# beilsme/rs-image-segmentation

Measured on AMD Instinct MI355X. Metric: Mpixel/s feature-extract+classify, higher is better.
Workload: dtype f32

## Files before the change

### profiles/code_object_diff.py

```python
#!/usr/bin/env python3
import json
import os
import re
import subprocess
import sys
import tempfile
from concurrent.futures import ThreadPoolExecutor

HIPCC = os.environ.get("HIPCC", "/opt/rocm/bin/hipcc")


def makefile_flags(csrc):
    text = open(os.path.join(csrc, "Makefile")).read()
    arch = re.search(r"^ARCH \?= *(\S+)", text, re.M).group(1)
    return re.search(r"^CXXFLAGS \?= *(.*)$", text, re.M).group(1).replace("$(ARCH)", arch).split()


def asm(csrc, f, tmp, tag):
    out = os.path.join(tmp, f"{tag}_{f}.s")
    subprocess.check_call([HIPCC, *makefile_flags(csrc), "--cuda-device-only", "-S", f, "-o", out], cwd=csrc, stderr=subprocess.DEVNULL)
    return open(out).read()


def demangle(names):
    p = subprocess.run(["c++filt"], input="\n".join(names), capture_output=True, text=True)
    return dict(zip(names, p.stdout.split("\n")))


def kernels(text):
    res = {}
    for m in re.finditer(r"^(\w+):\s*; @\1\n(.*?)^\s*\.end_amdhsa_kernel", text, re.S | re.M):
        ins = [ln.split(";")[0].strip() for ln in m.group(2).split("\n")]
        res[m.group(1)] = {"ins": [i for i in ins if i and not i.startswith(".")]}
    for m in re.finditer(r"- \.agpr_count:.*?\.name:\s+(\w+).*?\.wavefront_size", text, re.S):
        blk, name = m.group(0), m.group(1)
        if name in res:
            for key, field in (("vgprs", "vgpr_count"), ("agprs", "agpr_count"), ("sgprs", "sgpr_count"), ("lds", "group_segment_fixed_size"),
                               ("scratch", "private_segment_fixed_size"), ("wg", "max_flat_workgroup_size")):
                res[name][key] = int(re.search(r"\." + field + r":\s+(\d+)", blk).group(1))
    return res


def waves_per_simd(k):
    regs = -(-k["vgprs"] // 8) * 8 + -(-k["agprs"] // 8) * 8
    w = min(8, 512 // max(regs, 8))
    if k["lds"]:
        w = min(w, (160 * 1024 // k["lds"]) * -(-k["wg"] // 64) // 4)
    return w


def main():
    parent, new, outp, files = sys.argv[1], sys.argv[2], sys.argv[3], sys.argv[4:]
    table = []
    with tempfile.TemporaryDirectory() as tmp, ThreadPoolExecutor(8) as ex:
        jobs = {(t, f): ex.submit(asm, c, f, tmp, t) for f in files for t, c in (("parent", parent), ("new", new))
                if os.path.exists(os.path.join(c, f))}
        for f in files:
            if ("parent", f) not in jobs:
                kn = kernels(jobs[("new", f)].result())
                names = demangle(sorted(kn))
                for name in sorted(kn):
                    b = kn[name]
                    row = {"file": f, "kernel": names[name].split("(")[0].replace("void ", ""), "new_file": True}
                    for k in ("vgprs", "sgprs", "lds", "scratch"):
                        row[k] = [None, b[k]]
                    row["waves_per_simd"] = [None, waves_per_simd(b)]
                    row["instructions"] = [None, len(b["ins"])]
                    row["identical"] = None
                    row["within_the_rules"] = b["scratch"] == 0
                    table.append(row)
                    print("new  " + ("" if row["within_the_rules"] else "RULE ") + json.dumps(row))
                continue
            kp, kn = kernels(jobs[("parent", f)].result()), kernels(jobs[("new", f)].result())
            assert set(kp) == set(kn), (f, set(kp) ^ set(kn))
            names = demangle(sorted(kp))
            for name in sorted(kp):
                a, b = kp[name], kn[name]
                row = {"file": f, "kernel": names[name].split("(")[0].replace("void ", "")}
                for k in ("vgprs", "sgprs", "lds", "scratch"):
                    row[k] = [a[k], b[k]]
                row["waves_per_simd"] = [waves_per_simd(a), waves_per_simd(b)]
                row["instructions"] = [len(a["ins"]), len(b["ins"])]
                row["identical"] = a["ins"] == b["ins"]
                row["within_the_rules"] = b["scratch"] == 0 and a["lds"] == b["lds"] and row["waves_per_simd"][1] >= row["waves_per_simd"][0]
                table.append(row)
                print(("same " if row["identical"] else "DIFF ") + ("" if row["within_the_rules"] else "RULE ") + json.dumps(row))
    json.dump(table, open(outp, "w"), indent=1)


main()
```

### rs-image-segmentation_amd/csrc/k9_kmeans.hip

```cpp
#include <algorithm>
#include <chrono>
#include <cmath>
#include <type_traits>

#include "common.h"
#include "k9_kmeans.h"

template <typename T> constexpr bool lloyd_pipelined(int KMAX, int FR, bool UPDATE) { return KMAX <= 32 && (UPDATE || FR >= 16); }
template <typename T> constexpr bool kpp_pipelined(int NL, int FR) { return true; }
template <typename T> __device__ __forceinline__ int km_full_tiles(int64_t chunk0, int64_t n)
{
    const int64_t left = n - chunk0;
    if (left <= 0) return 0;
    const int64_t full = left / km_tile<T>();
    return full < KM_TILES_PER_CHUNK ? (int)full : KM_TILES_PER_CHUNK;
}

template <typename T>
__global__ __launch_bounds__(KM_THREADS) void km_minmax(planes_t pl, int64_t n, T *__restrict__ pmin, T *__restrict__ pmax)
{
    constexpr int PXL = vt<T>::PXL;
    const int f = blockIdx.y;
    T mn = (T)INFINITY, mx = (T)-INFINITY;
    for (int64_t base = ((int64_t)blockIdx.x * KM_THREADS + threadIdx.x) * PXL; base < n; base += (int64_t)gridDim.x * KM_THREADS * PXL) {
        T v[PXL];
// ... 48 lines not shown
            base += UNR * stride;
            if (!fits(base)) { consume(va); break; }
            request(vb, base);
            consume(va);
            base += UNR * stride;
            if (!fits(base)) { consume(vb); break; }
            request(va, base);
            consume(vb);
        }
    }
    for (; base < n; base += stride) {
        T v[PXL];
        load_px<T>(pl.p[f], base, n, v);
#pragma unroll
        for (int i = 0; i < PXL; i++)
            if (base + i < n) acc += to_fixed40((double)scaled<T>(v[i], sc, mnv));
    }
    __shared__ long long sacc[4];
    wg_put(sacc, wave_sum(acc));
    __syncthreads();
    if (threadIdx.x == 0) partial[(size_t)f * gridDim.x + blockIdx.x] = wg_sum(sacc);
}

template <typename T>
__global__ void km_gather_row(planes_t pl, int F, int64_t idx, const scaler_t<T> *__restrict__ sp, T *__restrict__ out)
{
    const int f = threadIdx.x;
    if (f < F) {
        T x = reinterpret_cast<const T *>(pl.p[f])[idx];
        out[f] = scaled<T>(x, sp->scale[f], sp->minv[f]) - sp->mean[f];
    }
}

#define KPP_MAXL 8
#define KPP_STRIDE (KPP_MAXL + 1)

template <typename T> __device__ __forceinline__ T kpp_close(double dot, double cc, double yy)
{
    double d = -2.0 * dot;
    d = d + cc;
    d = d + yy;
    const T dt = (T)d;
    return dt > (T)0 ? dt : (T)0;
}

template <typename T, int NL, int FR, int MODE>
__global__ __launch_bounds__(KM_THREADS) void km_kpp(planes_t pl, int F, int64_t n, const scaler_t<T> *__restrict__ sp,
                                                     const double *__restrict__ candT, const double *__restrict__ cc, int L,
                                                     T *__restrict__ closest, unsigned long long *__restrict__ partial, int64_t nchunks,
                                                     int store)
{
    constexpr int PXL = vt<T>::PXL;
    constexpr bool VAR = MODE == 0;
    constexpr bool PIPE = kpp_pipelined<T>(NL, FR);
    unsigned long long acc[NL];
#pragma unroll
    for (int l = 0; l < NL; l++) acc[l] = 0;
    long long vacc[VAR ? FR : 1];
#pragma unroll
    for (int f = 0; f < (VAR ? FR : 1); f++) vacc[f] = 0;
    const int64_t chunk0 = (int64_t)blockIdx.x * km_chunk<T>();
    auto request = [&](T (&x)[FR][PXL], T (&cl)[PXL], uint32_t off) {
#pragma unroll
        for (int f = 0; f < FR; f++) load_pxq<T>(pl, F, f, chunk0, off, x[f]);
        if constexpr (MODE == 2) load_pxf<T, true>(closest, chunk0 + off, n, cl);
    };
    auto tile_body = [&](auto full_t, auto roll_c, T (&x)[FR][PXL], T (&cl)[PXL], uint32_t off, uint32_t noff) {
        const int64_t base = chunk0 + off;
        constexpr bool FULL = decltype(full_t)::value;
        constexpr int ROLL = decltype(roll_c)::value;
        static_assert(ROLL == 0 || FULL, "only full tiles are requested ahead");
        if constexpr (ROLL == 0) {
#pragma unroll
            for (int f = 0; f < FR; f++) {
                if (f < F) load_pxf<T, FULL>(pl.p[f], base, n, x[f]);
                else {
#pragma unroll
                    for (int p = 0; p < PXL; p++) x[f][p] = (T)0;
                }
            }
#pragma unroll
            for (int p = 0; p < PXL; p++) cl[p] = (T)0;
            if constexpr (MODE == 2) load_pxf<T, FULL>(closest, base, n, cl);
        }
        double dot[NL][PXL], dotp[PXL], yy[PXL];
#pragma unroll
        for (int p = 0; p < PXL; p++) {
            yy[p] = 0.0;
            dotp[p] = 0.0;
#pragma unroll
            for (int l = 0; l < NL; l++) dot[l][p] = 0.0;
        }
#pragma unroll
        for (int f = 0; f < FR; f++) {
            if (f < F) {
                const T sc = sp->scale[f], mnv = sp->minv[f], me = sp->mean[f];
                double cd[NL];
#pragma unroll
                for (int l = 0; l < NL; l++) cd[l] = candT[f * KPP_STRIDE + l];
                const double cdp = candT[f * KPP_STRIDE + KPP_MAXL];
#pragma unroll
                for (int p = 0; p < PXL; p++) {
                    const T yt = scaled<T>(x[f][p], sc, mnv) - me;
                    if constexpr (VAR) {
                        const T dd = yt * yt;
                        if (FULL || base + p < n) vacc[f] += to_fixed40((double)dd);
                    }
                    const double y = (double)yt;
                    yy[p] = fma(y, y, yy[p]);
                    if constexpr (MODE != 0) dotp[p] = fma(cdp, y, dotp[p]);
#pragma unroll
                    for (int l = 0; l < NL; l++) dot[l][p] = fma(cd[l], y, dot[l][p]);
                }
            }
            if constexpr (ROLL == 1) load_pxq<T>(pl, F, f, chunk0, noff, x[f]);
        }
        if constexpr (MODE != 0) {
            const double ccp = cc[KPP_MAXL];
            bool moved = MODE != 2;
#pragma unroll
            for (int p = 0; p < PXL; p++) {
                T dt = kpp_close<T>(dotp[p], ccp, yy[p]);
                if constexpr (MODE == 2) {
                    moved = moved || dt < cl[p];
                    dt = cl[p] < dt ? cl[p] : dt;
                }
                cl[p] = dt;
            }
            if (!store) {
            } else if (FULL || base + PXL <= n) {
                if (moved) {
                    typename vt<T>::vec o;
                    if constexpr (PXL == 4) o = make_float4(cl[0], cl[1], cl[2], cl[3]);
                    else o = make_double2(cl[0], cl[1]);
                    *reinterpret_cast<typename vt<T>::vec *>(closest + base) = o;
                }
            } else {
                for (int p = 0; p < PXL; p++)
                    if (base + p < n) closest[base + p] = cl[p];
            }
        }
#pragma unroll
        for (int l = 0; l < NL; l++) {
            if (l < L) {
                const double ccl = cc[l];
#pragma unroll
                for (int p = 0; p < PXL; p++) {
                    T dt = kpp_close<T>(dot[l][p], ccl, yy[p]);
                    if constexpr (MODE != 0) dt = cl[p] < dt ? cl[p] : dt;
                    if (FULL || base + p < n) acc[l] += (unsigned long long)to_fixed40((double)dt);
                }
            }
        }
        if constexpr (ROLL == 1 && MODE == 2) load_pxf<T, true>(closest, chunk0 + noff, n, cl);
    };
    T x[FR][PXL], cl[PXL];
    auto at = [&](int t) { return (uint32_t)(t * km_tile<T>() + (int)threadIdx.x * PXL); };
    if constexpr (!PIPE) {
        for (int t = 0; t < KM_TILES_PER_CHUNK; t++) {
            const int64_t tbase = chunk0 + (int64_t)t * km_tile<T>();
            if (tbase >= n) break;
            if (tbase + km_tile<T>() <= n) tile_body(std::true_type{}, ic<0>(), x, cl, at(t), 0);
            else tile_body(std::false_type{}, ic<0>(), x, cl, at(t), 0);
        }
    } else {
        const int nfull = km_full_tiles<T>(chunk0, n);
        if (nfull > 0) {
            request(x, cl, at(0));
#pragma clang loop unroll(disable)
            for (int t = 0; t + 1 < nfull; t++) tile_body(std::true_type{}, ic<1>(), x, cl, at(t), at(t + 1));
            tile_body(std::true_type{}, ic<2>(), x, cl, at(nfull - 1), 0);
        }
        if (nfull < KM_TILES_PER_CHUNK && chunk0 + (int64_t)nfull * km_tile<T>() < n) tile_body(std::false_type{}, ic<0>(), x, cl, at(nfull), 0);
    }
    __shared__ unsigned long long sacc[4][NL];
#pragma unroll
    for (int l = 0; l < NL; l++) {
// ... 9 lines not shown
#pragma unroll
        for (int f = 0; f < FR; f++) {
            long long s = wave_sum(vacc[f]);
            if (lane_id() == 0) svar[threadIdx.x >> 6][f] = s;
        }
        __syncthreads();
        if ((int)threadIdx.x < F)
            partial[(size_t)(1 + threadIdx.x) * nchunks + blockIdx.x] =
                (unsigned long long)(svar[0][threadIdx.x] + svar[1][threadIdx.x] + svar[2][threadIdx.x] + svar[3][threadIdx.x]);
    }
}

struct kpp_sample_args {
    int64_t c0[KPP_MAXL], cn[KPP_MAXL], direct[KPP_MAXL];
    unsigned long long rem[KPP_MAXL];
    int mode[KPP_MAXL];
    int with_old;
    int64_t offset;
};
template <typename T>
__global__ __launch_bounds__(KM_THREADS) void km_kpp_chunkq(planes_t pl, int F, const scaler_t<T> *__restrict__ sp,
                                                            const double *__restrict__ candT, const double *__restrict__ cc,
                                                            const T *__restrict__ closest, const kpp_sample_args *__restrict__ ap,
                                                            unsigned long long *__restrict__ qv)
{
    const kpp_sample_args &a = *ap;
    const int l = blockIdx.y;
    if (a.mode[l] != 1) return;
    const int64_t c0 = a.c0[l], cn = a.cn[l];
    const int64_t i = (int64_t)blockIdx.x * KM_THREADS + threadIdx.x;
    if (i >= cn) return;
    const double ccp = cc[KPP_MAXL];
    double yy = 0.0, dotp = 0.0;
    for (int f = 0; f < F; f++) {
        const T xv = reinterpret_cast<const T *>(pl.p[f])[c0 + i];
        const T yt = scaled<T>(xv, sp->scale[f], sp->minv[f]) - sp->mean[f];
        const double y = (double)yt;
        yy = fma(y, y, yy);
        dotp = fma(candT[f * KPP_STRIDE + KPP_MAXL], y, dotp);
    }
    T dt = kpp_close<T>(dotp, ccp, yy);
    if (a.with_old) {
        const T c = closest[c0 + i];
        dt = c < dt ? c : dt;
    }
    qv[(size_t)l * km_chunk<T>() + i] = (unsigned long long)to_fixed40((double)dt);
}

template <typename T>
__global__ __launch_bounds__(KM_THREADS) void km_kpp_sample(planes_t pl, int F, const scaler_t<T> *__restrict__ sp,
                                                            const unsigned long long *__restrict__ qv, const kpp_sample_args *__restrict__ ap,
                                                            double *__restrict__ out)
{
    const kpp_sample_args &a = *ap;
// ... 782 lines not shown
    if (be == 0) e = -1074;
    else { m |= 1ull << 52; e = be - 1075; }
    const int sft = e + 40;
    if (sft >= 0) return (u128)m << sft;
    const int sh = -sft;
    if (sh >= 64) return (u128)1;
    const unsigned long long q = m >> sh, rem = m & ((1ull << sh) - 1ull);
    return (u128)q + (rem ? 1 : 0);
}

template <typename T>
__global__ __launch_bounds__(64) void kc_mean_pack(const km_state<T> *__restrict__ st, const T *__restrict__ row, int own0, long long *__restrict__ x)
{
    const int F = st->F, f = threadIdx.x;
    if (f >= F) return;
    if (st->n_local <= 0) { x[2 * f] = 0; x[2 * f + 1] = 0; }
    double rv = own0 ? (double)row[f] : 0.0;
    if (rv == 0.0) rv = 0.0;
    x[2 * F + f] = __double_as_longlong(rv);
}

template <typename T>
__global__ __launch_bounds__(KM_THREADS) void kc_mean_apply(km_state<T> *__restrict__ st, scaler_t<T> *__restrict__ sp, const long long *__restrict__ x,
                                                            double *__restrict__ candT)
{
    const int F = st->F;
    double *cc = candT + (size_t)KPP_STRIDE * RSSEG_MAX_FEATURES;
    for (int i = threadIdx.x; i < KPP_STRIDE * RSSEG_MAX_FEATURES + KPP_STRIDE; i += KM_THREADS) candT[i] = 0.0;
    __syncthreads();
    const T Nt = (T)st->N;
    if ((int)threadIdx.x < F) {
        const int f = threadIdx.x;
        const T sT = fixed_to_T<T>(limbs(x[2 * f], x[2 * f + 1]));
        const T m = sT / Nt;
        sp->mean[f] = m;
        st->mean[f] = m;
        const T raw = (T)__longlong_as_double(x[2 * F + f]);
        const T c0 = raw - m;
        st->C[0][f] = c0;
        candT[f * KPP_STRIDE] = (double)c0;
    }
    __syncthreads();
    if (threadIdx.x == 0) {
        double a = 0.0;
        for (int f = 0; f < F; f++) a = fma((double)st->C[0][f], (double)st->C[0][f], a);
        cc[0] = a;
    }
}

template <typename T>
__global__ __launch_bounds__(KM_THREADS) void kc_tol(km_state<T> *__restrict__ st, const long long *__restrict__ x)
{
    __shared__ T var[RSSEG_MAX_FEATURES];
    const int F = st->F;
    const T Nt = (T)st->N;
    if ((int)threadIdx.x < F) {
        const T sT = fixed_to_T<T>(limbs(x[2 * threadIdx.x], x[2 * threadIdx.x + 1]));
        var[threadIdx.x] = sT / Nt;
    }
    __syncthreads();
    if (threadIdx.x == 0) {
        const T m = np_pairwise_sum<T>(var, F);
        const T m2 = m / (T)F;
        st->tol = m2 * (T)st->tol_in;
        u128 total = 0;
        for (int r = 0; r < st->world; r++) {
            st->rank_tot[r] = kc_ulimbs(x[2 * F + 2 * r], x[2 * F + 2 * r + 1]);
            total += st->rank_tot[r];
        }
        st->current_pot = (T)((double)total * (1.0 / 1099511627776.0));
        st->best = 0;
    }
}

template <typename T> __device__ __forceinline__ void kc_pick_body(km_state<T> *st, int c, const long long *x);

template <typename T>
__global__ __launch_bounds__(KM_THREADS) void kc_targets(km_state<T> *st, int c, int pick_c, const unsigned long long *__restrict__ part,
                                                         double *__restrict__ candT, kpp_sample_args *__restrict__ sa_out, double *xbuf, long long *lim)
{
    if (pick_c > 0) kc_pick_body<T>(st, pick_c, lim);
    for (int i = threadIdx.x; i < KPP_MAXL * (1 + RSSEG_MAX_FEATURES); i += KM_THREADS) xbuf[i] = 0.0;
    for (int i = threadIdx.x; i < 2 * KPP_MAXL * RSSEG_MAX_RANKS; i += KM_THREADS)
        if (i < 2 * st->L * st->world) lim[i] = 0;
    const int F = st->F, L = st->L;
    double *cc = candT + (size_t)KPP_STRIDE * RSSEG_MAX_FEATURES;
    for (int i = threadIdx.x; i < KPP_STRIDE * RSSEG_MAX_FEATURES + KPP_STRIDE; i += KM_THREADS) candT[i] = 0.0;
    __syncthreads();
    if ((int)threadIdx.x < F) candT[threadIdx.x * KPP_STRIDE + KPP_MAXL] = (double)st->C[c - 1][threadIdx.x];
    if (threadIdx.x == 0) {
        double a = 0.0;
        for (int f = 0; f < F; f++) a = fma((double)st->C[c - 1][f], (double)st->C[c - 1][f], a);
        cc[KPP_MAXL] = a;
    }
    __shared__ kpp_sample_args sa;
    __shared__ u128 ssum[KM_THREADS];
    __shared__ u128 gsum[16];
    for (int i = threadIdx.x; i < (int)(sizeof(sa) / 4); i += KM_THREADS) reinterpret_cast<int *>(&sa)[i] = 0;
    const long long nchunks = st->nchunks, n = st->n_local;
    const unsigned long long *pre = part + (size_t)st->best * nchunks;
    const long long slice = (nchunks + KM_THREADS - 1) / KM_THREADS;
    {
        u128 mine = 0;
        const long long c_lo = (long long)threadIdx.x * slice, c_hi = c_lo + slice < nchunks ? c_lo + slice : nchunks;
        if (n > 0) {
            long long ch = c_lo;
            for (; ch + 8 <= c_hi; ch += 8) {
                unsigned long long v[8];
#pragma unroll
                for (int u = 0; u < 8; u++) v[u] = pre[ch + u];
#pragma unroll
                for (int u = 0; u < 8; u++) mine += v[u];
            }
            for (; ch < c_hi; ch++) mine += pre[ch];
        }
        ssum[threadIdx.x] = mine;
// ... 223 lines not shown
                if (update) {
                    RSCHK(set_max_dyn_lds(ctx, (const void *)km_lloyd_blk<T, KM, true>, lds));
                    hipLaunchKernelGGL((km_lloyd_blk<T, KM, true>), grid, block, lds, ctx->stream, pl, F, k, n, sp, cenT, csq, labels, partial,
                                       nchunks, ncopies, done);
                } else {
                    hipLaunchKernelGGL((km_lloyd_blk<T, KM, false>), grid, block, 0, ctx->stream, pl, F, k, n, sp, cenT, csq, labels, partial,
                                       nchunks, ncopies, done);
                }
            } else {
                if (update) {
                    RSCHK(set_max_dyn_lds(ctx, (const void *)km_lloyd<T, KM, FR, true>, lds));
                    hipLaunchKernelGGL((km_lloyd<T, KM, FR, true>), grid, block, lds, ctx->stream, pl, F, k, n, sp, cenT, csq, labels, partial,
                                       nchunks, ncopies, done, (int32_t *)nullptr);
                } else {
                    hipLaunchKernelGGL((km_lloyd<T, KM, FR, false>), grid, block, 0, ctx->stream, pl, F, k, n, sp, cenT, csq, labels, partial,
                                       nchunks, ncopies, done, out32);
                }
            }
            return RSSEG_OK;
        });
    });
}

template <typename T>
void launch_kpp(rsseg_ctx *ctx, int64_t nchunks, planes_t pl, int F, int64_t n, const scaler_t<T> *sp, const double *cand, const double *cc,
                int L, int mode, bool last, T *closest, unsigned long long *partial)
{
    auto go = [&](auto nl_c, auto mode_c) {
        constexpr int NL = decltype(nl_c)::value, MODE = decltype(mode_c)::value;
        with_width(km_width(F), [&](auto fr_c) {
            constexpr int FR = decltype(fr_c)::value;
            const dim3 grid((unsigned)nchunks), block(KM_THREADS);
            if constexpr (FR != KM_BLOCKED) {
                hipLaunchKernelGGL((km_kpp<T, NL, FR, MODE>), grid, block, 0, ctx->stream, pl, F, n, sp, cand, cc, L, closest, partial, nchunks,
                                   last ? 0 : 1);
            } else {
                hipLaunchKernelGGL((km_kpp_blk<T, NL, MODE>), grid, block, 0, ctx->stream, pl, F, n, sp, cand, cc, L, closest, partial, nchunks,
                                   last ? 0 : 1);
                if constexpr (MODE == 0)
                    hipLaunchKernelGGL((km_var<T>), dim3((unsigned)nchunks, F), block, 0, ctx->stream, pl, n, sp, partial, nchunks);
            }
        });
    };
    if (mode == 0) go(ic<1>(), ic<0>());
    else if (L <= 4) mode == 1 ? go(ic<4>(), ic<1>()) : go(ic<4>(), ic<2>());
    else mode == 1 ? go(ic<8>(), ic<1>()) : go(ic<8>(), ic<2>());
}

template <typename T>
void launch_farthest(rsseg_ctx *ctx, int KMAX, int64_t nchunks, planes_t pl, int F, int64_t n, int64_t offset, const scaler_t<T> *sp,
                     const T *cenT, const uint8_t *labels, const taken_t &tk, T *pdist, long long *pidx)
{
    with_kmax(KMAX, [&](auto kmax_c) {
        with_width(km_width(F), [&](auto fr_c) {
            hipLaunchKernelGGL((km_farthest<T, decltype(kmax_c)::value, decltype(fr_c)::value>), dim3((unsigned)nchunks), dim3(KM_THREADS), 0,
                               ctx->stream, pl, F, n, offset, sp, cenT, labels, tk, pdist, pidx);
        });
    });
}

constexpr size_t LIM_OFF = ((sizeof(double) * KPP_MAXL * (1 + RSSEG_MAX_FEATURES)) + 511) & ~(size_t)511;
constexpr size_t UP_SLOT = 64 * 1024;

template <typename T> struct km_fit {
    static constexpr int CHUNK = km_chunk<T>();
    rsseg_ctx *ctx = nullptr;
    hipStream_t st = nullptr;
    planes_t pl;
    int max_iter = 0;
    int F = 0, k = 0, KMAX = 0, L = 0, M = 0, nblk = 0;
    int64_t n = 0, nchunks = 0, N = 0, offset = 0;
    int64_t n_all[RSSEG_MAX_RANKS] = {0};
    int last_rank = 0;
    struct {
        scaler_t<T> *sp;
        T *cen, *csq;
        double *cand, *cc;
        T *row;
        unsigned long long *qv;
        long long *red;
        kpp_sample_args *sa;
        long long *redsave;
        km_state<T> *lst;
        T *mm;
        long long *mom, *part;
        T *closest;
        uint8_t *lab;
    } d;
    long long *x = nullptr;
    size_t pin_main = 0;
    unsigned up_i = 0, up_since_sync = 0;
    long long up_epoch = 0;
    int ncopies = KM_COPIES;
    size_t lds = 0;
    scaler_t<T> sp;
    T C[RSSEG_MAX_CLUSTERS][RSSEG_MAX_FEATURES];
    int64_t init_idx[RSSEG_MAX_CLUSTERS];
    T tol = (T)0;
    int it = 0, relocated = 0;
    bool strict = false;

    int setup(rsseg_ctx *c, int F_, int64_t n_, int k_, int max_iter_)
    {
        ctx = c;
        st = c->stream;
        F = F_, n = n_, k = k_, max_iter = max_iter_;
        KMAX = km_kmax(k);
        L = 2 + (int)std::log((double)k);
        if (L > KPP_MAXL) return rs_fail(ctx, RSSEG_ERR_UNSUPPORTED, "kmeans: too many local trials");
        M = KMAX * F + KMAX + 1;
        nchunks = std::max<int64_t>(1, ceil_div64(n, CHUNK));
        nblk = (int)std::min<int64_t>(2048, std::max<int64_t>(1, ceil_div64(n, (int64_t)KM_THREADS * vt<T>::PXL)));
        while (ncopies > 1 && sizeof(long long) * (size_t)ncopies * km_copy_stride(KMAX, F) > 48 * 1024) ncopies >>= 1;
        lds = sizeof(long long) * (size_t)ncopies * km_copy_stride(KMAX, F);
        if (lds > 150 * 1024) return rs_fail(ctx, RSSEG_ERR_UNSUPPORTED, "kmeans: F=%d, k=%d needs %zu B of LDS", F, k, lds);
        return RSSEG_OK;
    }

    int layout(const void *const *d_planes)
    {
        const size_t x_bytes = sizeof(long long) * std::max<size_t>({(size_t)2 * M, (size_t)3 * F, (size_t)2 * F + 2 * (size_t)ctx->world,
                                                                     LIM_OFF / sizeof(long long) + 2 * (size_t)L * ctx->world});
        if (ctx->comm_on && x_bytes > ctx->comm_bytes) return rs_fail(ctx, RSSEG_ERR_COMM, "kmeans: comm buffer too small (%zu > %zu)", x_bytes, ctx->comm_bytes);
        size_t off = 0;
        auto carve = [&](size_t bytes) { size_t o = off; off = (off + bytes + 255) & ~(size_t)255; return o; };
        const size_t o_sp = carve(sizeof(scaler_t<T>));
        const size_t o_cen = carve(sizeof(T) * ((size_t)KMAX * RSSEG_MAX_FEATURES + KMAX));
        const size_t o_cand = carve(sizeof(double) * ((size_t)KPP_STRIDE * RSSEG_MAX_FEATURES + KPP_STRIDE));
        const size_t o_row = carve(sizeof(T) * RSSEG_MAX_FEATURES);
        const size_t o_qv = carve(sizeof(unsigned long long) * KPP_MAXL * (size_t)CHUNK);
        const size_t o_red = carve(x_bytes);
        const size_t o_sa = carve(sizeof(kpp_sample_args));
        const size_t o_redsave = carve(sizeof(long long) * 2 * M);
        const size_t o_lst = carve(sizeof(km_state<T>));
        const size_t o_mm = carve(sizeof(T) * 2 * (size_t)nblk * F);
        const size_t o_mom = carve(sizeof(long long) * (size_t)nblk * F);
        const size_t o_part = carve(sizeof(long long) * std::max<size_t>((size_t)M, KPP_MAXL) * (size_t)nchunks);
        const size_t o_closest = carve((sizeof(T) * (size_t)std::max<int64_t>(n, 1) + 255) & ~(size_t)255);
        const size_t o_lab = carve((size_t)std::max<int64_t>(n, 1) + 64);
        RSCHK(ws_reserve(ctx, off));
        char *ws = ctx->d_ws;
        d.sp = (scaler_t<T> *)(ws + o_sp);
        d.cen = (T *)(ws + o_cen);
        d.csq = d.cen + (size_t)KMAX * RSSEG_MAX_FEATURES;
        d.cand = (double *)(ws + o_cand);
        d.cc = d.cand + (size_t)KPP_STRIDE * RSSEG_MAX_FEATURES;
        d.row = (T *)(ws + o_row);
        d.qv = (unsigned long long *)(ws + o_qv);
        d.red = (long long *)(ws + o_red);
        d.sa = (kpp_sample_args *)(ws + o_sa);
        d.redsave = (long long *)(ws + o_redsave);
        d.lst = (km_state<T> *)(ws + o_lst);
        d.mm = (T *)(ws + o_mm);
        d.mom = (long long *)(ws + o_mom);
        d.part = (long long *)(ws + o_part);
        d.closest = (T *)(ws + o_closest);
        d.lab = (uint8_t *)(ws + o_lab);
        x = ctx->comm_on ? (long long *)ctx->d_comm : d.red;
        const size_t pin_need = std::max<size_t>({sizeof(T) * 2 * (size_t)nblk * F, sizeof(long long) * (size_t)nblk * F + sizeof(double) * RSSEG_MAX_FEATURES + 64,
                                                  sizeof(long long) * (size_t)std::max(KPP_MAXL, F + 1) * (size_t)nchunks, sizeof(T) * (size_t)CHUNK,
                                                  sizeof(long long) * 2 * (size_t)M + sizeof(km_state<T>), (size_t)65536});
        pin_main = (pin_need + 255) & ~(size_t)255;
        RSCHK(pin_reserve(ctx, pin_main + 4 * UP_SLOT));
        up_epoch = ctx->host_syncs;
        memset(&pl, 0, sizeof(pl));
        for (int f = 0; f < F; f++) {
            if (n > 0 && (!d_planes[f] || ((uintptr_t)d_planes[f] & 15))) return rs_fail(ctx, RSSEG_ERR_INVALID, "kmeans: plane %d null or not 16-byte aligned", f);
            pl.p[f] = d_planes[f];
        }
        return RSSEG_OK;
    }

    hipError_t upload(void *dst, const void *src, size_t bytes)
    {
        if (ctx->host_syncs != up_epoch) { up_epoch = ctx->host_syncs; up_since_sync = 0; }
        if (up_since_sync == 4) {
            const hipError_t e = rs_sync(ctx);
            if (e != hipSuccess) return e;
            up_epoch = ctx->host_syncs;
// ... 58 lines not shown
    {
        {
            mt19937 rng(seed);
            km_state<T> hs;
            memset(&hs, 0, sizeof(hs));
            const double u0 = rng.random_sample();
            init_idx[0] = uniform_choice(N, std::is_same<T, float>::value ? RSSEG_F32 : RSSEG_F64, u0);
            if (init_idx[0] >= N) init_idx[0] = N - 1;
            for (int i = 0; i < (k - 1) * L; i++) hs.uniforms[i] = rng.random_sample();
            hs.init_idx[0] = init_idx[0];
            hs.max_iter = max_iter;
            for (int r = 0; r < ctx->world; r++) hs.n_all[r] = n_all[r];
            hs.N = N; hs.offset = offset; hs.n_local = n; hs.nchunks = nchunks;
            hs.rank = ctx->rank; hs.world = ctx->world; hs.k = k; hs.F = F; hs.L = L; hs.last_rank = last_rank;
            hs.tol_in = tol_in;
            static_assert(sizeof(hs) <= UP_SLOT, "upload slot too small");
            HIPCHK(ctx, upload(d.lst, &hs, sizeof(hs)));
        }
        const int64_t li0 = init_idx[0] - offset;
        const bool own0 = li0 >= 0 && li0 < n;
        if (n > 0) {
            {
                prof_scope ps(ctx, "moment");
                hipLaunchKernelGGL((km_moment<T>), dim3(nblk, F), dim3(KM_THREADS), 0, st, pl, n, d.sp, d.mom);
            }
            if (own0) hipLaunchKernelGGL((km_gather_row<T>), dim3(1), dim3(64), 0, st, pl, F, li0, d.sp, d.row);
            hipLaunchKernelGGL(km_reduce_cols, dim3(F), dim3(KM_THREADS), 0, st, (const long long *)d.mom, (int64_t)nblk, x, (const int *)nullptr, 1, 0);
        }
        hipLaunchKernelGGL((kc_mean_pack<T>), dim3(1), dim3(64), 0, st, (const km_state<T> *)d.lst, (const T *)d.row, own0 ? 1 : 0, x);
        HIPCHK(ctx, hipGetLastError());
        RSCHK(comm_allreduce_dev(ctx, 0, 3 * F, RSSEG_I64, RSSEG_SUM));
        hipLaunchKernelGGL((kc_mean_apply<T>), dim3(1), dim3(KM_THREADS), 0, st, d.lst, d.sp, (const long long *)x, d.cand);
        HIPCHK(ctx, hipGetLastError());
        return RSSEG_OK;
    }

    int kpp_rounds()
    {
        if (n > 0) {
            prof_scope ps(ctx, "kpp");
            launch_kpp<T>(ctx, nchunks, pl, F, n, d.sp, d.cand, d.cc, 1, 0, false, d.closest, (unsigned long long *)d.part);
        }
        HIPCHK(ctx, hipGetLastError());
        HIPCHK(ctx, hipMemsetAsync(x, 0, sizeof(long long) * (2 * (size_t)F + 2 * (size_t)ctx->world), st));
        if (n > 0) {
            hipLaunchKernelGGL(km_reduce_cols, dim3(F), dim3(KM_THREADS), 0, st, (const long long *)d.part + nchunks, nchunks, x, (const int *)nullptr, 1, 0);
            hipLaunchKernelGGL(km_reduce_cols, dim3(1), dim3(KM_THREADS), 0, st, (const long long *)d.part, nchunks, x + 2 * F, (const int *)nullptr, 1, ctx->rank);
        }
        HIPCHK(ctx, hipGetLastError());
        RSCHK(comm_allreduce_dev(ctx, 0, 2 * F + 2 * ctx->world, RSSEG_I64, RSSEG_SUM));
        hipLaunchKernelGGL((kc_tol<T>), dim3(1), dim3(KM_THREADS), 0, st, d.lst, (const long long *)x);
        HIPCHK(ctx, hipGetLastError());
        double *xbuf = (double *)x;
        long long *lim = (long long *)((char *)x + LIM_OFF);
        for (int c = 1; c < k; c++) {
            hipLaunchKernelGGL((kc_targets<T>), dim3(1), dim3(KM_THREADS), 0, st, d.lst, c, c > 1 ? c - 1 : 0, (const unsigned long long *)d.part, d.cand, d.sa,
                               xbuf, lim);
            if (n > 0) {
                hipLaunchKernelGGL((km_kpp_chunkq<T>), dim3((unsigned)(CHUNK / KM_THREADS), L), dim3(KM_THREADS), 0, st, pl, F, d.sp, d.cand, d.cc,
                                   (const T *)d.closest, (const kpp_sample_args *)d.sa, d.qv);
                hipLaunchKernelGGL((km_kpp_sample<T>), dim3(L), dim3(KM_THREADS), 0, st, pl, F, d.sp, (const unsigned long long *)d.qv, (const kpp_sample_args *)d.sa, xbuf);
            }
            HIPCHK(ctx, hipGetLastError());
            RSCHK(comm_allreduce_dev(ctx, 0, (int64_t)L * (1 + RSSEG_MAX_FEATURES), RSSEG_F64, RSSEG_SUM));
            hipLaunchKernelGGL((kc_cands<T>), dim3(1), dim3(KM_THREADS), 0, st, d.lst, (const double *)xbuf, d.cand);
            if (n > 0) {
                prof_scope ps(ctx, "kpp");
                launch_kpp<T>(ctx, nchunks, pl, F, n, d.sp, d.cand, d.cc, L, c > 1 ? 2 : 1, c == k - 1, d.closest, (unsigned long long *)d.part);
            }
            HIPCHK(ctx, hipGetLastError());
            if (n > 0) hipLaunchKernelGGL(km_reduce_cols, dim3(L), dim3(KM_THREADS), 0, st, (const long long *)d.part, nchunks, lim, (const int *)nullptr, ctx->world, ctx->rank);
            RSCHK(comm_allreduce_dev(ctx, (int64_t)LIM_OFF, 2 * (int64_t)L * ctx->world, RSSEG_I64, RSSEG_SUM));
        }
        if (k > 1) {
            hipLaunchKernelGGL((kc_pick<T>), dim3(1), dim3(KM_THREADS), 0, st, d.lst, k - 1, (const long long *)lim);
            HIPCHK(ctx, hipGetLastError());
        }
        return RSSEG_OK;
    }

    int lloyd_sweep(bool update, bool from_state, bool force, int32_t *out32 = nullptr, bool track = true)
    {
        if (!from_state) {
            T cenT[RSSEG_MAX_FEATURES * RSSEG_MAX_CLUSTERS + RSSEG_MAX_CLUSTERS];
            T *csq = cenT + (size_t)KMAX * RSSEG_MAX_FEATURES;
            memset(cenT, 0, sizeof(cenT));
            for (int j = 0; j < k; j++) {
                T a = (T)0;
                for (int f = 0; f < F; f++) {
                    cenT[f * KMAX + j] = C[j][f];
                    a = std::is_same<T, float>::value ? (T)fmaf((float)C[j][f], (float)C[j][f], (float)a) : (T)std::fma((double)C[j][f], (double)C[j][f], (double)a);
// ... 335 lines not shown
```

Baseline: 3864.

## Recompute k-means++ closest distances from chosen centers instead of streaming the closest plane

```diff
diff --git a/profiles/code_object_diff.py b/profiles/code_object_diff.py
--- a/profiles/code_object_diff.py
+++ b/profiles/code_object_diff.py
@@ -27,10 +27,21 @@
     return dict(zip(names, p.stdout.split("\n")))
 
 
+def short(demangled):
+    return demangled.split("(")[0].replace("void ", "")
+
+
+def by_name(kn):
+    names = demangle(sorted(kn))
+    out = {short(names[m]): v for m, v in kn.items()}
+    assert len(out) == len(kn), "two kernels share a name"
+    return out
+
+
 def kernels(text):
     res = {}
     for m in re.finditer(r"^(\w+):\s*; @\1\n(.*?)^\s*\.end_amdhsa_kernel", text, re.S | re.M):
-        ins = [ln.split(";")[0].strip() for ln in m.group(2).split("\n")]
+        ins = [re.sub(r"\.L(\w+?)\d+_(\d+)", r".L\1_\2", ln.split(";")[0].strip()) for ln in m.group(2).split("\n")]
         res[m.group(1)] = {"ins": [i for i in ins if i and not i.startswith(".")]}
     for m in re.finditer(r"- \.agpr_count:.*?\.name:\s+(\w+).*?\.wavefront_size", text, re.S):
         blk, name = m.group(0), m.group(1)
@@ -71,13 +82,23 @@
                     table.append(row)
                     print("new  " + ("" if row["within_the_rules"] else "RULE ") + json.dumps(row))
                 continue
-            kp, kn = kernels(jobs[("parent", f)].result()), kernels(jobs[("new", f)].result())
-            assert set(kp) == set(kn), (f, set(kp) ^ set(kn))
-            names = demangle(sorted(kp))
+            kp, kn = by_name(kernels(jobs[("parent", f)].result())), by_name(kernels(jobs[("new", f)].result()))
+            assert set(kp) <= set(kn), (f, set(kp) - set(kn))
+            for name in sorted(set(kn) - set(kp)):
+                b = kn[name]
+                row = {"file": f, "kernel": name, "new_kernel": True}
+                for k in ("vgprs", "agprs", "sgprs", "lds", "scratch"):
+                    row[k] = [None, b[k]]
+                row["waves_per_simd"] = [None, waves_per_simd(b)]
+                row["instructions"] = [None, len(b["ins"])]
+                row["identical"] = None
+                row["within_the_rules"] = b["scratch"] == 0
+                table.append(row)
+                print("new  " + ("" if row["within_the_rules"] else "RULE ") + json.dumps(row))
             for name in sorted(kp):
                 a, b = kp[name], kn[name]
-                row = {"file": f, "kernel": names[name].split("(")[0].replace("void ", "")}
-                for k in ("vgprs", "sgprs", "lds", "scratch"):
+                row = {"file": f, "kernel": name}
+                for k in ("vgprs", "agprs", "sgprs", "lds", "scratch"):
                     row[k] = [a[k], b[k]]
                 row["waves_per_simd"] = [waves_per_simd(a), waves_per_simd(b)]
                 row["instructions"] = [len(a["ins"]), len(b["ins"])]
diff --git a/rs-image-segmentation_amd/csrc/k9_kmeans.hip b/rs-image-segmentation_amd/csrc/k9_kmeans.hip
--- a/rs-image-segmentation_amd/csrc/k9_kmeans.hip
+++ b/rs-image-segmentation_amd/csrc/k9_kmeans.hip
@@ -1,6 +1,7 @@
 #include <algorithm>
 #include <chrono>
 #include <cmath>
+#include <cstdlib>
 #include <type_traits>
 
 #include "common.h"
@@ -95,6 +96,63 @@
     if (threadIdx.x == 0) partial[(size_t)f * gridDim.x + blockIdx.x] = wg_sum(sacc);
 }
 
+template <typename T, int FR>
+__global__ __launch_bounds__(KM_THREADS) void km_moment_chunk(planes_t pl, int F, int64_t n, const scaler_t<T> *__restrict__ sp,
+                                                              long long *__restrict__ partial, int64_t nchunks)
+{
+    constexpr int PXL = vt<T>::PXL;
+    long long acc[FR];
+#pragma unroll
+    for (int f = 0; f < FR; f++) acc[f] = 0;
+    const int64_t chunk0 = (int64_t)blockIdx.x * km_chunk<T>();
+    auto tile_body = [&](auto full_t, auto roll_c, T (&x)[FR][PXL], uint32_t off, uint32_t noff) {
+        const int64_t base = chunk0 + off;
+        constexpr bool FULL = decltype(full_t)::value;
+        constexpr int ROLL = decltype(roll_c)::value;
+        static_assert(ROLL == 0 || FULL, "only full tiles are requested ahead");
+        if constexpr (ROLL == 0) {
+#pragma unroll
+            for (int f = 0; f < FR; f++) {
+                if (f < F) load_pxf<T, FULL>(pl.p[f], base, n, x[f]);
+                else {
+#pragma unroll
+                    for (int p = 0; p < PXL; p++) x[f][p] = (T)0;
+                }
+            }
+        }
+#pragma unroll
+        for (int f = 0; f < FR; f++) {
+            if (f < F) {
+                const T sc = sp->scale[f], mnv = sp->minv[f];
+#pragma unroll
+                for (int p = 0; p < PXL; p++)
+                    if (FULL || base + p < n) acc[f] += to_fixed40((double)scaled<T>(x[f][p], sc, mnv));
+            }
+            if constexpr (ROLL == 1) load_pxq<T>(pl, F, f, chunk0, noff, x[f]);
+        }
+    };
+    T x[FR][PXL];
+    auto at = [&](int t) { return (uint32_t)(t * km_tile<T>() + (int)threadIdx.x * PXL); };
+    const int nfull = km_full_tiles<T>(chunk0, n);
+    if (nfull > 0) {
+#pragma unroll
+        for (int f = 0; f < FR; f++) load_pxq<T>(pl, F, f, chunk0, at(0), x[f]);
+#pragma clang loop unroll(disable)
+        for (int t = 0; t + 1 < nfull; t++) tile_body(std::true_type{}, ic<1>(), x, at(t), at(t + 1));
+        tile_body(std::true_type{}, ic<2>(), x, at(nfull - 1), 0);
+    }
+    if (nfull < KM_TILES_PER_CHUNK && chunk0 + (int64_t)nfull * km_tile<T>() < n) tile_body(std::false_type{}, ic<0>(), x, at(nfull), 0);
+    __shared__ long long sacc[4][FR];
+#pragma unroll
+    for (int f = 0; f < FR; f++) {
+        long long s = wave_sum(acc[f]);
+        if (lane_id() == 0) sacc[threadIdx.x >> 6][f] = s;
+    }
+    __syncthreads();
+    if ((int)threadIdx.x < F)
+        partial[(size_t)threadIdx.x * nchunks + blockIdx.x] = sacc[0][threadIdx.x] + sacc[1][threadIdx.x] + sacc[2][threadIdx.x] + sacc[3][threadIdx.x];
+}
+
 template <typename T>
 __global__ void km_gather_row(planes_t pl, int F, int64_t idx, const scaler_t<T> *__restrict__ sp, T *__restrict__ out)
 {
@@ -107,6 +165,13 @@
 
 #define KPP_MAXL 8
 #define KPP_STRIDE (KPP_MAXL + 1)
+
+#define KPP_MAXREC 4
+#define KPP_RECOMPUTE 3
+template <typename T> constexpr bool kpp_recompute(int NL, int FR)
+{
+    return !(std::is_same<T, double>::value && NL == 4 && FR == 8) && !(std::is_same<T, float>::value && NL == 8 && FR == 32);
+}
 
 template <typename T> __device__ __forceinline__ T kpp_close(double dot, double cc, double yy)
 {
@@ -121,10 +186,13 @@
 __global__ __launch_bounds__(KM_THREADS) void km_kpp(planes_t pl, int F, int64_t n, const scaler_t<T> *__restrict__ sp,
                                                      const double *__restrict__ candT, const double *__restrict__ cc, int L,
                                                      T *__restrict__ closest, unsigned long long *__restrict__ partial, int64_t nchunks,
-                                                     int store)
-{
+                                                     int store, const double *__restrict__ chosT, int nrec)
+{
+    static_assert(MODE != 3 || kpp_recompute<T>(NL, FR), "MODE 3 exists only where MODE 2 is the recompute form");
     constexpr int PXL = vt<T>::PXL;
     constexpr bool VAR = MODE == 0;
+    constexpr bool REC = MODE == 2 && kpp_recompute<T>(NL, FR);
+    constexpr bool FOLD = MODE == 3 || (MODE == 2 && !REC);
     constexpr bool PIPE = kpp_pipelined<T>(NL, FR);
     unsigned long long acc[NL];
 #pragma unroll
@@ -136,7 +204,7 @@
     auto request = [&](T (&x)[FR][PXL], T (&cl)[PXL], uint32_t off) {
 #pragma unroll
         for (int f = 0; f < FR; f++) load_pxq<T>(pl, F, f, chunk0, off, x[f]);
-        if constexpr (MODE == 2) load_pxf<T, true>(closest, chunk0 + off, n, cl);
+        if constexpr (FOLD) load_pxf<T, true>(closest, chunk0 + off, n, cl);
     };
     auto tile_body = [&](auto full_t, auto roll_c, T (&x)[FR][PXL], T (&cl)[PXL], uint32_t off, uint32_t noff) {
         const int64_t base = chunk0 + off;
@@ -154,7 +222,82 @@
             }
 #pragma unroll
             for (int p = 0; p < PXL; p++) cl[p] = (T)0;
-            if constexpr (MODE == 2) load_pxf<T, FULL>(closest, base, n, cl);
+            if constexpr (FOLD) load_pxf<T, FULL>(closest, base, n, cl);
+        }
+        if constexpr (REC) {
+            double dot[NL][PXL], dc[KPP_MAXREC][PXL], yy[PXL];
+#pragma unroll
+            for (int p = 0; p < PXL; p++) {
+                yy[p] = 0.0;
+#pragma unroll
+                for (int l = 0; l < NL; l++) dot[l][p] = 0.0;
+#pragma unroll
+                for (int j = 0; j < KPP_MAXREC; j++) dc[j][p] = 0.0;
+            }
+#pragma unroll
+            for (int f = 0; f < FR; f++) {
+                if (f < F) {
+                    const T sc = sp->scale[f], mnv = sp->minv[f], me = sp->mean[f];
+                    double cd[NL], cj[KPP_MAXREC];
+#pragma unroll
+                    for (int l = 0; l < NL; l++) cd[l] = candT[f * KPP_STRIDE + l];
+#pragma unroll
+                    for (int j = 0; j < KPP_MAXREC; j++) cj[j] = chosT[f * KPP_MAXREC + j];
+                    double y[PXL];
+#pragma unroll
+                    for (int p = 0; p < PXL; p++) {
+                        y[p] = (double)(scaled<T>(x[f][p], sc, mnv) - me);
+                        yy[p] = fma(y[p], y[p], yy[p]);
+#pragma unroll
+                        for (int l = 0; l < NL; l++) dot[l][p] = fma(cd[l], y[p], dot[l][p]);
+                    }
+#pragma unroll
+                    for (int j = 0; j < KPP_MAXREC; j++) {
+                        if (j < nrec) {
+#pragma unroll
+                            for (int p = 0; p < PXL; p++) dc[j][p] = fma(cj[j], y[p], dc[j][p]);
+                        }
+                    }
+                }
+                if constexpr (ROLL == 1) load_pxq<T>(pl, F, f, chunk0, noff, x[f]);
+            }
+            {
+                const double *chcc = chosT + (size_t)KPP_MAXREC * RSSEG_MAX_FEATURES;
+#pragma unroll
+                for (int j = 0; j < KPP_MAXREC; j++) {
+                    if (j == 0 || j < nrec) {
+                        const double ccj = chcc[j];
+#pragma unroll
+                        for (int p = 0; p < PXL; p++) {
+                            const T dt = kpp_close<T>(dc[j][p], ccj, yy[p]);
+                            cl[p] = j == 0 || dt < cl[p] ? dt : cl[p];
+                        }
+                    }
+                }
+            }
+            if (!store) {
+            } else if (FULL || base + PXL <= n) {
+                typename vt<T>::vec o;
+                if constexpr (PXL == 4) o = make_float4(cl[0], cl[1], cl[2], cl[3]);
+                else o = make_double2(cl[0], cl[1]);
+                *reinterpret_cast<typename vt<T>::vec *>(closest + base) = o;
+            } else {
+                for (int p = 0; p < PXL; p++)
+                    if (base + p < n) closest[base + p] = cl[p];
+            }
+#pragma unroll
+            for (int l = 0; l < NL; l++) {
+                if (l < L) {
+                    const double ccl = cc[l];
+#pragma unroll
+                    for (int p = 0; p < PXL; p++) {
+                        T dt = kpp_close<T>(dot[l][p], ccl, yy[p]);
+                        dt = cl[p] < dt ? cl[p] : dt;
+                        if (FULL || base + p < n) acc[l] += (unsigned long long)to_fixed40((double)dt);
+                    }
+                }
+            }
+            return;
         }
         double dot[NL][PXL], dotp[PXL], yy[PXL];
 #pragma unroll
@@ -190,11 +333,11 @@
         }
         if constexpr (MODE != 0) {
             const double ccp = cc[KPP_MAXL];
-            bool moved = MODE != 2;
+            bool moved = !FOLD;
 #pragma unroll
             for (int p = 0; p < PXL; p++) {
                 T dt = kpp_close<T>(dotp[p], ccp, yy[p]);
-                if constexpr (MODE == 2) {
+                if constexpr (FOLD) {
                     moved = moved || dt < cl[p];
                     dt = cl[p] < dt ? cl[p] : dt;
                 }
@@ -225,7 +368,7 @@
                 }
             }
         }
-        if constexpr (ROLL == 1 && MODE == 2) load_pxf<T, true>(closest, chunk0 + noff, n, cl);
+        if constexpr (ROLL == 1 && FOLD) load_pxf<T, true>(closest, chunk0 + noff, n, cl);
     };
     T x[FR][PXL], cl[PXL];
     auto at = [&](int t) { return (uint32_t)(t * km_tile<T>() + (int)threadIdx.x * PXL); };
@@ -281,7 +424,7 @@
 __global__ __launch_bounds__(KM_THREADS) void km_kpp_chunkq(planes_t pl, int F, const scaler_t<T> *__restrict__ sp,
                                                             const double *__restrict__ candT, const double *__restrict__ cc,
                                                             const T *__restrict__ closest, const kpp_sample_args *__restrict__ ap,
-                                                            unsigned long long *__restrict__ qv)
+                                                            unsigned long long *__restrict__ qv, const double *__restrict__ chosT, int nrec)
 {
     const kpp_sample_args &a = *ap;
     const int l = blockIdx.y;
@@ -289,6 +432,30 @@
     const int64_t c0 = a.c0[l], cn = a.cn[l];
     const int64_t i = (int64_t)blockIdx.x * KM_THREADS + threadIdx.x;
     if (i >= cn) return;
+    if (nrec > 0) {
+        double yy = 0.0, dc[KPP_MAXREC];
+#pragma unroll
+        for (int j = 0; j < KPP_MAXREC; j++) dc[j] = 0.0;
+        for (int f = 0; f < F; f++) {
+            const T xv = reinterpret_cast<const T *>(pl.p[f])[c0 + i];
+            const T yt = scaled<T>(xv, sp->scale[f], sp->minv[f]) - sp->mean[f];
+            const double y = (double)yt;
+            yy = fma(y, y, yy);
+#pragma unroll
+            for (int j = 0; j < KPP_MAXREC; j++)
+                if (j < nrec) dc[j] = fma(chosT[f * KPP_MAXREC + j], y, dc[j]);
+        }
+        const double *chcc = chosT + (size_t)KPP_MAXREC * RSSEG_MAX_FEATURES;
+        T best = kpp_close<T>(dc[0], chcc[0], yy);
+#pragma unroll
+        for (int j = 1; j < KPP_MAXREC; j++)
+            if (j < nrec) {
+                const T dt = kpp_close<T>(dc[j], chcc[j], yy);
+                best = dt < best ? dt : best;
+            }
+        qv[(size_t)l * km_chunk<T>() + i] = (unsigned long long)to_fixed40((double)best);
+        return;
+    }
     const double ccp = cc[KPP_MAXL];
     double yy = 0.0, dotp = 0.0;
     for (int f = 0; f < F; f++) {
@@ -1117,11 +1284,13 @@
 
 template <typename T>
 __global__ __launch_bounds__(KM_THREADS) void kc_mean_apply(km_state<T> *__restrict__ st, scaler_t<T> *__restrict__ sp, const long long *__restrict__ x,
-                                                            double *__restrict__ candT)
+                                                            double *__restrict__ candT, double *__restrict__ chosT)
 {
     const int F = st->F;
     double *cc = candT + (size_t)KPP_STRIDE * RSSEG_MAX_FEATURES;
+    double *chcc = chosT + (size_t)KPP_MAXREC * RSSEG_MAX_FEATURES;
     for (int i = threadIdx.x; i < KPP_STRIDE * RSSEG_MAX_FEATURES + KPP_STRIDE; i += KM_THREADS) candT[i] = 0.0;
+    for (int i = threadIdx.x; i < KPP_MAXREC * RSSEG_MAX_FEATURES + KPP_MAXREC; i += KM_THREADS) chosT[i] = 0.0;
     __syncthreads();
     const T Nt = (T)st->N;
     if ((int)threadIdx.x < F) {
@@ -1134,12 +1303,14 @@
         const T c0 = raw - m;
         st->C[0][f] = c0;
         candT[f * KPP_STRIDE] = (double)c0;
+        chosT[f * KPP_MAXREC] = (double)c0;
     }
     __syncthreads();
     if (threadIdx.x == 0) {
         double a = 0.0;
         for (int f = 0; f < F; f++) a = fma((double)st->C[0][f], (double)st->C[0][f], a);
         cc[0] = a;
+        chcc[0] = a;
     }
 }
 
@@ -1172,7 +1343,8 @@
 
 template <typename T>
 __global__ __launch_bounds__(KM_THREADS) void kc_targets(km_state<T> *st, int c, int pick_c, const unsigned long long *__restrict__ part,
-                                                         double *__restrict__ candT, kpp_sample_args *__restrict__ sa_out, double *xbuf, long long *lim)
+                                                         double *__restrict__ candT, kpp_sample_args *__restrict__ sa_out, double *xbuf, long long *lim,
+                                                         double *__restrict__ chosT)
 {
     if (pick_c > 0) kc_pick_body<T>(st, pick_c, lim);
     for (int i = threadIdx.x; i < KPP_MAXL * (1 + RSSEG_MAX_FEATURES); i += KM_THREADS) xbuf[i] = 0.0;
@@ -1182,11 +1354,16 @@
     double *cc = candT + (size_t)KPP_STRIDE * RSSEG_MAX_FEATURES;
     for (int i = threadIdx.x; i < KPP_STRIDE * RSSEG_MAX_FEATURES + KPP_STRIDE; i += KM_THREADS) candT[i] = 0.0;
     __syncthreads();
-    if ((int)threadIdx.x < F) candT[threadIdx.x * KPP_STRIDE + KPP_MAXL] = (double)st->C[c - 1][threadIdx.x];
+    const bool slot = c - 1 < KPP_MAXREC;
+    if ((int)threadIdx.x < F) {
+        candT[threadIdx.x * KPP_STRIDE + KPP_MAXL] = (double)st->C[c - 1][threadIdx.x];
+        if (slot) chosT[threadIdx.x * KPP_MAXREC + c - 1] = (double)st->C[c - 1][threadIdx.x];
+    }
     if (threadIdx.x == 0) {
         double a = 0.0;
         for (int f = 0; f < F; f++) a = fma((double)st->C[c - 1][f], (double)st->C[c - 1][f], a);
         cc[KPP_MAXL] = a;
+        if (slot) chosT[(size_t)KPP_MAXREC * RSSEG_MAX_FEATURES + c - 1] = a;
     }
     __shared__ kpp_sample_args sa;
     __shared__ u128 ssum[KM_THREADS];
@@ -1456,9 +1633,20 @@
     });
 }
 
+template <typename T> bool kpp_has_recompute(int L, int F)
+{
+    const int NL = L <= 4 ? 4 : 8;
+    switch (km_width(F)) {
+    case 8: return kpp_recompute<T>(NL, 8);
+    case 16: return kpp_recompute<T>(NL, 16);
+    case 32: return kpp_recompute<T>(NL, 32);
+    default: return false;
+    }
+}
+
 template <typename T>
 void launch_kpp(rsseg_ctx *ctx, int64_t nchunks, planes_t pl, int F, int64_t n, const scaler_t<T> *sp, const double *cand, const double *cc,
-                int L, int mode, bool last, T *closest, unsigned long long *partial)
+                int L, int mode, bool store, T *closest, unsigned long long *partial, const double *chos, int nrec)
 {
     auto go = [&](auto nl_c, auto mode_c) {
         constexpr int NL = decltype(nl_c)::value, MODE = decltype(mode_c)::value;
@@ -1466,16 +1654,27 @@
             constexpr int FR = decltype(fr_c)::value;
             const dim3 grid((unsigned)nchunks), block(KM_THREADS);
             if constexpr (FR != KM_BLOCKED) {
-                hipLaunchKernelGGL((km_kpp<T, NL, FR, MODE>), grid, block, 0, ctx->stream, pl, F, n, sp, cand, cc, L, closest, partial, nchunks,
-                                   last ? 0 : 1);
+                constexpr bool REC = kpp_recompute<T>(NL, FR);
+                if constexpr (MODE == 2 && REC) {
+                    if (nrec > 0)
+                        hipLaunchKernelGGL((km_kpp<T, NL, FR, 2>), grid, block, 0, ctx->stream, pl, F, n, sp, cand, cc, L, closest, partial, nchunks,
+                                           store ? 1 : 0, chos, nrec);
+                    else
+                        hipLaunchKernelGGL((km_kpp<T, NL, FR, 3>), grid, block, 0, ctx->stream, pl, F, n, sp, cand, cc, L, closest, partial, nchunks,
+                                           store ? 1 : 0, chos, 0);
+                } else {
+                    hipLaunchKernelGGL((km_kpp<T, NL, FR, MODE>), grid, block, 0, ctx->stream, pl, F, n, sp, cand, cc, L, closest, partial, nchunks,
+                                       store ? 1 : 0, chos, 0);
+                }
             } else {
                 hipLaunchKernelGGL((km_kpp_blk<T, NL, MODE>), grid, block, 0, ctx->stream, pl, F, n, sp, cand, cc, L, closest, partial, nchunks,
-                                   last ? 0 : 1);
+                                   store ? 1 : 0);
                 if constexpr (MODE == 0)
                     hipLaunchKernelGGL((km_var<T>), dim3((unsigned)nchunks, F), block, 0, ctx->stream, pl, n, sp, partial, nchunks);
             }
         });
     };
+    if (nrec > 0) mode = 2;
     if (mode == 0) go(ic<1>(), ic<0>());
     else if (L <= 4) mode == 1 ? go(ic<4>(), ic<1>()) : go(ic<4>(), ic<2>());
     else mode == 1 ? go(ic<8>(), ic<1>()) : go(ic<8>(), ic<2>());
@@ -1503,6 +1702,7 @@
     planes_t pl;
     int max_iter = 0;
     int F = 0, k = 0, KMAX = 0, L = 0, M = 0, nblk = 0;
+    int kpp_depth = 0;
     int64_t n = 0, nchunks = 0, N = 0, offset = 0;
     int64_t n_all[RSSEG_MAX_RANKS] = {0};
     int last_rank = 0;
@@ -1510,6 +1710,7 @@
         scaler_t<T> *sp;
         T *cen, *csq;
         double *cand, *cc;
+        double *chos;
         T *row;
         unsigned long long *qv;
         long long *red;
@@ -1543,6 +1744,11 @@
         L = 2 + (int)std::log((double)k);
         if (L > KPP_MAXL) return rs_fail(ctx, RSSEG_ERR_UNSUPPORTED, "kmeans: too many local trials");
         M = KMAX * F + KMAX + 1;
+        kpp_depth = kpp_has_recompute<T>(L, F) ? KPP_RECOMPUTE : 0;
+        if (const char *e = getenv("RSSEG_KPP_RECOMPUTE")) {
+            const int v = atoi(e);
+            if (kpp_depth > 0 && v >= 0 && v <= KPP_MAXREC) kpp_depth = v;
+        }
         nchunks = std::max<int64_t>(1, ceil_div64(n, CHUNK));
         nblk = (int)std::min<int64_t>(2048, std::max<int64_t>(1, ceil_div64(n, (int64_t)KM_THREADS * vt<T>::PXL)));
         while (ncopies > 1 && sizeof(long long) * (size_t)ncopies * km_copy_stride(KMAX, F) > 48 * 1024) ncopies >>= 1;
@@ -1561,6 +1767,7 @@
         const size_t o_sp = carve(sizeof(scaler_t<T>));
         const size_t o_cen = carve(sizeof(T) * ((size_t)KMAX * RSSEG_MAX_FEATURES + KMAX));
         const size_t o_cand = carve(sizeof(double) * ((size_t)KPP_STRIDE * RSSEG_MAX_FEATURES + KPP_STRIDE));
+        const size_t o_chos = carve(sizeof(double) * ((size_t)KPP_MAXREC * RSSEG_MAX_FEATURES + KPP_MAXREC));
         const size_t o_row = carve(sizeof(T) * RSSEG_MAX_FEATURES);
         const size_t o_qv = carve(sizeof(unsigned long long) * KPP_MAXL * (size_t)CHUNK);
         const size_t o_red = carve(x_bytes);
@@ -1570,7 +1777,8 @@
         const size_t o_mm = carve(sizeof(T) * 2 * (size_t)nblk * F);
         const size_t o_mom = carve(sizeof(long long) * (size_t)nblk * F);
         const size_t o_part = carve(sizeof(long long) * std::max<size_t>((size_t)M, KPP_MAXL) * (size_t)nchunks);
-        const size_t o_closest = carve((sizeof(T) * (size_t)std::max<int64_t>(n, 1) + 255) & ~(size_t)255);
+        const bool plane = k - 1 > kpp_depth;
+        const size_t o_closest = plane ? carve((sizeof(T) * (size_t)std::max<int64_t>(n, 1) + 255) & ~(size_t)255) : 0;
         const size_t o_lab = carve((size_t)std::max<int64_t>(n, 1) + 64);
         RSCHK(ws_reserve(ctx, off));
         char *ws = ctx->d_ws;
@@ -1588,7 +1796,8 @@
         d.mm = (T *)(ws + o_mm);
         d.mom = (long long *)(ws + o_mom);
         d.part = (long long *)(ws + o_part);
-        d.closest = (T *)(ws + o_closest);
+        d.closest = plane ? (T *)(ws + o_closest) : nullptr;
+        d.chos = (double *)(ws + o_chos);
         d.lab = (uint8_t *)(ws + o_lab);
         x = ctx->comm_on ? (long long *)ctx->d_comm : d.red;
         const size_t pin_need = std::max<size_t>({sizeof(T) * 2 * (size_t)nblk * F, sizeof(long long) * (size_t)nblk * F + sizeof(double) * RSSEG_MAX_FEATURES + 64,
@@ -1693,15 +1902,24 @@
         if (n > 0) {
             {
                 prof_scope ps(ctx, "moment");
-                hipLaunchKernelGGL((km_moment<T>), dim3(nblk, F), dim3(KM_THREADS), 0, st, pl, n, d.sp, d.mom);
+                with_width(km_width(F), [&](auto fr_c) {
+                    constexpr int FR = decltype(fr_c)::value;
+                    if constexpr (FR != KM_BLOCKED)
+                        hipLaunchKernelGGL((km_moment_chunk<T, FR>), dim3((unsigned)nchunks), dim3(KM_THREADS), 0, st, pl, F, n, d.sp, d.part, nchunks);
+                    else
+                        hipLaunchKernelGGL((km_moment<T>), dim3(nblk, F), dim3(KM_THREADS), 0, st, pl, n, d.sp, d.mom);
+                });
             }
             if (own0) hipLaunchKernelGGL((km_gather_row<T>), dim3(1), dim3(64), 0, st, pl, F, li0, d.sp, d.row);
-            hipLaunchKernelGGL(km_reduce_cols, dim3(F), dim3(KM_THREADS), 0, st, (const long long *)d.mom, (int64_t)nblk, x, (const int *)nullptr, 1, 0);
+            if (km_width(F) != KM_BLOCKED)
+                hipLaunchKernelGGL(km_reduce_cols, dim3(F), dim3(KM_THREADS), 0, st, (const long long *)d.part, nchunks, x, (const int *)nullptr, 1, 0);
+            else
+                hipLaunchKernelGGL(km_reduce_cols, dim3(F), dim3(KM_THREADS), 0, st, (const long long *)d.mom, (int64_t)nblk, x, (const int *)nullptr, 1, 0);
         }
         hipLaunchKernelGGL((kc_mean_pack<T>), dim3(1), dim3(64), 0, st, (const km_state<T> *)d.lst, (const T *)d.row, own0 ? 1 : 0, x);
         HIPCHK(ctx, hipGetLastError());
         RSCHK(comm_allreduce_dev(ctx, 0, 3 * F, RSSEG_I64, RSSEG_SUM));
-        hipLaunchKernelGGL((kc_mean_apply<T>), dim3(1), dim3(KM_THREADS), 0, st, d.lst, d.sp, (const long long *)x, d.cand);
+        hipLaunchKernelGGL((kc_mean_apply<T>), dim3(1), dim3(KM_THREADS), 0, st, d.lst, d.sp, (const long long *)x, d.cand, d.chos);
         HIPCHK(ctx, hipGetLastError());
         return RSSEG_OK;
     }
@@ -1710,7 +1928,7 @@
     {
         if (n > 0) {
             prof_scope ps(ctx, "kpp");
-            launch_kpp<T>(ctx, nchunks, pl, F, n, d.sp, d.cand, d.cc, 1, 0, false, d.closest, (unsigned long long *)d.part);
+            launch_kpp<T>(ctx, nchunks, pl, F, n, d.sp, d.cand, d.cc, 1, 0, true, d.closest, (unsigned long long *)d.part, d.chos, 0);
         }
         HIPCHK(ctx, hipGetLastError());
         HIPCHK(ctx, hipMemsetAsync(x, 0, sizeof(long long) * (2 * (size_t)F + 2 * (size_t)ctx->world), st));
@@ -1725,11 +1943,13 @@
         double *xbuf = (double *)x;
         long long *lim = (long long *)((char *)x + LIM_OFF);
         for (int c = 1; c < k; c++) {
+            const int nrec = c <= kpp_depth ? c : 0;
+            const bool store = nrec > 0 ? (c == kpp_depth && c < k - 1) : c < k - 1;
             hipLaunchKernelGGL((kc_targets<T>), dim3(1), dim3(KM_THREADS), 0, st, d.lst, c, c > 1 ? c - 1 : 0, (const unsigned long long *)d.part, d.cand, d.sa,
-                               xbuf, lim);
+                               xbuf, lim, d.chos);
             if (n > 0) {
                 hipLaunchKernelGGL((km_kpp_chunkq<T>), dim3((unsigned)(CHUNK / KM_THREADS), L), dim3(KM_THREADS), 0, st, pl, F, d.sp, d.cand, d.cc,
-                                   (const T *)d.closest, (const kpp_sample_args *)d.sa, d.qv);
+                                   (const T *)d.closest, (const kpp_sample_args *)d.sa, d.qv, (const double *)d.chos, nrec);
                 hipLaunchKernelGGL((km_kpp_sample<T>), dim3(L), dim3(KM_THREADS), 0, st, pl, F, d.sp, (const unsigned long long *)d.qv, (const kpp_sample_args *)d.sa, xbuf);
             }
             HIPCHK(ctx, hipGetLastError());
@@ -1737,7 +1957,7 @@
             hipLaunchKernelGGL((kc_cands<T>), dim3(1), dim3(KM_THREADS), 0, st, d.lst, (const double *)xbuf, d.cand);
             if (n > 0) {
                 prof_scope ps(ctx, "kpp");
-                launch_kpp<T>(ctx, nchunks, pl, F, n, d.sp, d.cand, d.cc, L, c > 1 ? 2 : 1, c == k - 1, d.closest, (unsigned long long *)d.part);
+                launch_kpp<T>(ctx, nchunks, pl, F, n, d.sp, d.cand, d.cc, L, c > 1 ? 2 : 1, store, d.closest, (unsigned long long *)d.part, d.chos, nrec);
             }
             HIPCHK(ctx, hipGetLastError());
             if (n > 0) hipLaunchKernelGGL(km_reduce_cols, dim3(L), dim3(KM_THREADS), 0, st, (const long long *)d.part, nchunks, lim, (const int *)nullptr, ctx->world, ctx->rank);
```

Result: faster. 3936 (median of 6 runs) (+1.9%).
